# mynameisfiber/baton

Measured on NVIDIA H100. Metric: federated local samples/sec (whole box), ResNet-18 FedAvg, synthetic non-IID 32x32 shards, higher is better.
Workload: dtype bf16

## Files before the change

baton_b200/csrc/bindings.cpp:

```cpp
#include <ATen/cuda/CUDAContext.h>
#include <c10/cuda/CUDAGuard.h>
#include <torch/extension.h>

#include <optional>
#include <vector>

#include "launch.h"

namespace {

inline cudaStream_t cur_stream() { return at::cuda::getCurrentCUDAStream().stream(); }
inline void check(int rc, const char* what) {
  TORCH_CHECK(rc == 0, "baton_b200::", what, " failed with code ", rc,
              rc > 0 ? std::string(" (") + cudaGetErrorString(static_cast<cudaError_t>(rc)) + ")" : std::string());
}
inline const void* cptr(const at::Tensor& t) { return t.data_ptr(); }
inline void* ptr(at::Tensor& t) { return t.data_ptr(); }
template <class T>
inline T* opt_ptr(const std::optional<at::Tensor>& t) {
  return (t.has_value() && t->defined()) ? reinterpret_cast<T*>(t->data_ptr()) : nullptr;
}
#define CHECK_CUDA(x) TORCH_CHECK((x).is_cuda(), #x " must be a CUDA tensor")

inline const float* prox_anchor(const std::optional<at::Tensor>& anchor, int64_t numel, const at::Tensor& hyper) {
// ... 187 lines not shown
                    int64_t pad, int64_t ho, int64_t wo, int64_t cluster_k, int64_t force_bn,
                    const std::optional<at::Tensor>& col_stats, const std::optional<at::Tensor>& bn_scale,
                    const std::optional<at::Tensor>& bn_shift, const std::optional<at::Tensor>& residual, bool bn_relu) {
  CHECK_CUDA(x); CHECK_CUDA(w); CHECK_CUDA(y);
  TORCH_CHECK(x.scalar_type() == at::kBFloat16 && w.scalar_type() == at::kBFloat16 && y.scalar_type() == at::kBFloat16 &&
              x.dim() == 4 && x.is_contiguous() && w.is_contiguous() && y.is_contiguous());
  TORCH_CHECK(y.numel() == x.size(0) * ho * wo * w.size(0), "conv_igemm_fwd: y must hold [N*Ho*Wo, Cout] elements");
  const c10::cuda::CUDAGuard guard(x.device());
  const std::optional<B200AffineEpilogue> affine =
      affine_epilogue(bn_scale, bn_shift, residual, bn_relu, x.size(0) * ho * wo, w.size(0));
  const int rc = b200_conv_igemm_fwd(cptr(x), cptr(w), ptr(y), static_cast<int>(x.size(0)), static_cast<int>(x.size(1)),
                                     static_cast<int>(x.size(2)), static_cast<int>(x.size(3)), static_cast<int>(w.size(0)),
                                     static_cast<int>(kh), static_cast<int>(kw), static_cast<int>(stride),
                                     static_cast<int>(pad), static_cast<int>(ho), static_cast<int>(wo),
                                     static_cast<int>(cluster_k), static_cast<int>(force_bn), opt_ptr<float>(col_stats),
                                     affine ? &*affine : nullptr, cur_stream());
  if (rc == -2 || rc == B200_AFFINE_EPILOGUE_DECLINED) return false;
  check(rc, "conv_igemm_fwd");
  return true;
}
bool conv_igemm_dgrad(const at::Tensor& dy, const at::Tensor& w, at::Tensor dx, int64_t kh, int64_t kw, int64_t pad,
                      int64_t cluster_k, int64_t force_bn) {
  CHECK_CUDA(dy); CHECK_CUDA(w); CHECK_CUDA(dx);
  TORCH_CHECK(dy.scalar_type() == at::kBFloat16 && w.scalar_type() == at::kBFloat16 && dx.scalar_type() == at::kBFloat16 &&
              dy.dim() == 4 && dx.dim() == 4 && dy.is_contiguous() && w.is_contiguous() && dx.is_contiguous());
  const c10::cuda::CUDAGuard guard(dy.device());
  const int rc = b200_conv_igemm_dgrad(cptr(dy), cptr(w), ptr(dx), static_cast<int>(dx.size(0)), static_cast<int>(dx.size(1)),
                                       static_cast<int>(dx.size(2)), static_cast<int>(dx.size(3)), static_cast<int>(dy.size(3)),
                                       static_cast<int>(kh), static_cast<int>(kw), static_cast<int>(pad),
                                       static_cast<int>(dy.size(1)), static_cast<int>(dy.size(2)),
                                       static_cast<int>(cluster_k), static_cast<int>(force_bn), cur_stream());
  if (rc == -2) return false;
  check(rc, "conv_igemm_dgrad");
  return true;
}
bool conv_halo(const at::Tensor& src, const at::Tensor& w, at::Tensor out, bool dgrad, int64_t mc,
               const std::optional<at::Tensor>& col_stats) {
  CHECK_CUDA(src); CHECK_CUDA(w); CHECK_CUDA(out);
  TORCH_CHECK(src.scalar_type() == at::kBFloat16 && w.scalar_type() == at::kBFloat16 && out.scalar_type() == at::kBFloat16 &&
              src.dim() == 4 && src.size(3) == 64 && src.is_contiguous() && w.is_contiguous() && out.is_contiguous());
  const int64_t rows = src.size(0) * src.size(1) * src.size(2);
  TORCH_CHECK(rows > 0 && out.numel() % rows == 0, "conv_halo: out must hold [N*H*W, Nout] elements");
  const int64_t nout = out.numel() / rows;
  TORCH_CHECK(w.numel() == (dgrad ? 64 * 9 * nout : nout * 9 * 64), "conv_halo: w must be [Cout, 9*Cin]");
  TORCH_CHECK(dgrad ? !col_stats.has_value()
                    : (!col_stats.has_value() || (col_stats->scalar_type() == at::kFloat && col_stats->numel() >= 2 * nout)),
              "conv_halo: col_stats is a [2 Cout] fp32 buffer of the forward");
  const c10::cuda::CUDAGuard guard(src.device());
  const int rc = b200_conv_halo(cptr(src), cptr(w), ptr(out), static_cast<int>(src.size(0)), static_cast<int>(src.size(1)),
                                static_cast<int>(src.size(2)), static_cast<int>(nout), dgrad ? 1 : 0,
                                static_cast<int>(mc), opt_ptr<float>(col_stats), cur_stream());
  if (rc == -2) return false;
  check(rc, "conv_halo");
  return true;
}
bool conv_igemm_dgrad_s2(const at::Tensor& dy, const at::Tensor& w, at::Tensor dx, int64_t kh, int64_t kw,
                         const std::vector<int64_t>& ntaps, const std::vector<int64_t>& taps, int64_t force_bn) {
  CHECK_CUDA(dy); CHECK_CUDA(w); CHECK_CUDA(dx);
  TORCH_CHECK(dy.scalar_type() == at::kBFloat16 && w.scalar_type() == at::kBFloat16 && dx.scalar_type() == at::kBFloat16 &&
              dy.dim() == 4 && dx.dim() == 4 && dy.is_contiguous() && w.is_contiguous() && dx.is_contiguous());
  TORCH_CHECK(ntaps.size() == 4 && taps.size() == 16, "conv_igemm_dgrad_s2: 4 classes x 4 taps");
  int nt[4], tw[16];
  for (int i = 0; i < 4; ++i) nt[i] = static_cast<int>(ntaps[i]);
  for (int i = 0; i < 16; ++i) tw[i] = static_cast<int>(taps[i]);
  const c10::cuda::CUDAGuard guard(dy.device());
  const int rc = b200_conv_igemm_dgrad_s2(cptr(dy), cptr(w), ptr(dx), static_cast<int>(dx.size(0)),
                                          static_cast<int>(dx.size(1)), static_cast<int>(dx.size(2)),
                                          static_cast<int>(dx.size(3)), static_cast<int>(dy.size(3)), static_cast<int>(kh),
                                          static_cast<int>(kw), static_cast<int>(dy.size(1)), static_cast<int>(dy.size(2)),
                                          nt, tw, static_cast<int>(force_bn), cur_stream());
  if (rc == -2) return false;
  check(rc, "conv_igemm_dgrad_s2");
  return true;
}
bool conv_igemm_wgrad(const at::Tensor& dy, const at::Tensor& x, at::Tensor dw, int64_t cout, int64_t kh, int64_t kw,
                      int64_t stride, int64_t pad, int64_t ho, int64_t wo, int64_t split_k, int64_t force_bn,
                      const std::optional<at::Tensor>& sgd_theta, const std::optional<at::Tensor>& sgd_theta_bf16,
                      const std::optional<at::Tensor>& sgd_mom, const std::optional<at::Tensor>& sgd_hyper,
                      bool sgd_nesterov, const std::optional<at::Tensor>& sgd_anchor,
                      const std::optional<at::Tensor>& sgd_corr, const std::optional<at::Tensor>& sgd_v) {
  CHECK_CUDA(dy); CHECK_CUDA(x); CHECK_CUDA(dw);
  TORCH_CHECK(x.scalar_type() == at::kBFloat16 && dy.scalar_type() == at::kBFloat16 && dw.scalar_type() == at::kFloat &&
              x.dim() == 4 && x.is_contiguous() && dy.is_contiguous());
  const c10::cuda::CUDAGuard guard(x.device());
  const std::optional<B200SgdEpilogue> sgd =
      sgd_epilogue(sgd_theta, sgd_theta_bf16, sgd_mom, sgd_hyper, sgd_nesterov, sgd_anchor, sgd_corr, sgd_v);
  const int rc = b200_conv_igemm_wgrad(cptr(dy), cptr(x), dw.data_ptr<float>(), static_cast<int>(x.size(0)),
                                       static_cast<int>(x.size(1)), static_cast<int>(x.size(2)), static_cast<int>(x.size(3)),
                                       static_cast<int>(cout), static_cast<int>(kh), static_cast<int>(kw),
                                       static_cast<int>(stride), static_cast<int>(pad), static_cast<int>(ho),
                                       static_cast<int>(wo), static_cast<int>(split_k), static_cast<int>(force_bn),
                                       sgd ? &*sgd : nullptr, cur_stream());
  if (rc == -2 || rc == B200_SGD_EPILOGUE_DECLINED) return false;
  check(rc, "conv_igemm_wgrad");
  return true;
}

void gemm_fp8(const at::Tensor& a, const at::Tensor& b, at::Tensor d, const std::optional<at::Tensor>& bias,
              const std::optional<at::Tensor>& sfa, const std::optional<at::Tensor>& sfb, int64_t M, int64_t N, int64_t K,
              int64_t lda, int64_t ldb, int64_t ldd, int64_t act, int64_t split_k, bool accumulate, double alpha) {
  CHECK_CUDA(a); CHECK_CUDA(b); CHECK_CUDA(d);
  TORCH_CHECK(a.element_size() == 1 && b.element_size() == 1, "gemm_fp8 operands must be 1-byte (e4m3)");
  const c10::cuda::CUDAGuard guard(a.device());
  check(b200_gemm_fp8(cptr(a), cptr(b), ptr(d), opt_ptr<const float>(bias), opt_ptr<const void>(sfa),
                      opt_ptr<const void>(sfb), M, N, K, lda, ldb, ldd, d.scalar_type() == at::kFloat, act, split_k,
                      accumulate, static_cast<float>(alpha), cur_stream()),
// ... 758 lines not shown
                                       opt_ptr<float>(logits_out), static_cast<int>(x.size(0)), static_cast<int>(x.size(1)),
                                       static_cast<int>(w.size(0)), static_cast<float>(grad_scale), cur_stream());
  if (rc == -2) return false;
  check(rc, "linear_xent_head");
  return true;
}
bool linear_xent_eval(const at::Tensor& x, const at::Tensor& w, const std::optional<at::Tensor>& bias, const at::Tensor& target,
                      at::Tensor loss_acc, const std::optional<at::Tensor>& logits_out) {
  CHECK_CUDA(x);
  TORCH_CHECK(x.scalar_type() == at::kBFloat16 && w.scalar_type() == at::kBFloat16 && x.dim() == 2 && w.dim() == 2 &&
              x.is_contiguous() && w.is_contiguous() && x.size(1) == w.size(1));
  TORCH_CHECK(target.scalar_type() == at::kLong && target.numel() >= x.size(0) && loss_acc.scalar_type() == at::kFloat &&
              loss_acc.numel() >= 2);
  TORCH_CHECK(!bias.has_value() || (bias->scalar_type() == at::kFloat && bias->numel() == w.size(0)));
  TORCH_CHECK(!logits_out.has_value() || (logits_out->scalar_type() == at::kFloat && logits_out->is_contiguous() &&
                                          logits_out->numel() == x.size(0) * w.size(0)));
  const c10::cuda::CUDAGuard guard(x.device());
  const int rc = b200_linear_xent_eval(x.data_ptr(), w.data_ptr(), opt_ptr<const float>(bias),
                                       reinterpret_cast<const long long*>(target.data_ptr<int64_t>()),
                                       loss_acc.data_ptr<float>(), opt_ptr<float>(logits_out), static_cast<int>(x.size(0)),
                                       static_cast<int>(x.size(1)), static_cast<int>(w.size(0)), cur_stream());
  if (rc == -2) return false;
  check(rc, "linear_xent_eval");
  return true;
}
void mse(const at::Tensor& pred, const at::Tensor& target, const std::optional<at::Tensor>& dpred, at::Tensor loss_acc,
         double grad_scale) {
  CHECK_CUDA(pred);
  TORCH_CHECK(target.scalar_type() == at::kFloat && target.numel() == pred.numel());
  const c10::cuda::CUDAGuard guard(pred.device());
  const int in32 = pred.scalar_type() == at::kFloat;
  const int out32 = dpred.has_value() && dpred->defined() && dpred->scalar_type() == at::kFloat;
  check(b200_mse(pred.data_ptr(), in32, target.data_ptr<float>(), opt_ptr<void>(dpred), out32,
                 loss_acc.data_ptr<float>(), pred.numel(), static_cast<float>(grad_scale), cur_stream()),
        "mse");
}

}

PYBIND11_MODULE(TORCH_EXTENSION_NAME, m) {
  m.doc() = "baton_b200 sm_90a kernels";
  m.attr("MAX_RANKS") = B200_MAX_RANKS;
  m.def("gemm", &gemm);
  m.def("trace_set", &trace_set);
  m.def("attention_fwd", &attention_fwd);
  m.def("attention_bwd", &attention_bwd);
  m.def("bn_bwd_cluster", &bn_bwd_cluster);
  m.def("im2col_tma_probe", &im2col_tma_probe);
  m.def("conv_igemm_fwd", &conv_igemm_fwd);
  m.def("conv_igemm_wgrad", &conv_igemm_wgrad);
  m.def("conv_igemm_dgrad", &conv_igemm_dgrad);
  m.def("conv_igemm_dgrad_s2", &conv_igemm_dgrad_s2);
  m.def("conv_halo", &conv_halo);
  m.def("gemm_batched", &gemm_batched);
  m.def("gemm_fp8", &gemm_fp8);
  m.def("quant_mx_rows", &quant_mx_rows);
  m.def("quant_mx_cols", &quant_mx_cols);
  m.def("fused_sgd", &fused_sgd);
  m.def("fused_sgd_segments", &fused_sgd_segments);
  m.def("weighted_sum", &weighted_sum);
  m.def("fold_client", &fold_client);
  m.def("scaffold_corr", &scaffold_corr);
  m.def("scaffold_dc", &scaffold_dc);
  m.def("cast", &cast);
  m.def("gather_rows", &gather_rows);
  m.def("colsum", &colsum);
  m.def("add_bf16", &add_bf16);
  m.def("relu_bwd", &relu_bwd);
  m.def("gelu", &gelu);
  m.def("gelu_bwd", &gelu_bwd);
  m.def("pad_rows", &pad_rows);
  m.def("embedding_bwd", &embedding_bwd);
  m.def("fedavg_allreduce", &fedavg_allreduce);
  m.def("fedavg_allreduce_robust", &fedavg_allreduce_robust);
  m.def("fedavg_allreduce_krum", &fedavg_allreduce_krum);
  m.attr("KRUM_MAX_CTAS") = B200_KRUM_MAX_CTAS;
  m.attr("KRUM_PAIRS") = B200_KRUM_PAIRS;
  m.attr("KRUM_REPORT") = B200_KRUM_REPORT;
  m.def("fedavg_allreduce_topk", &fedavg_allreduce_topk);
  m.def("fedavg_allreduce_local", &fedavg_allreduce_local);
  m.def("topk_pack", &topk_pack);
  m.def("topk_fold", &topk_fold);
  m.def("nonzero_pack", &nonzero_pack);
  m.def("topk_work_words", [](int64_t n) { return static_cast<int64_t>(B200_TOPK_WORK_WORDS(n)); });
  m.def("pack_client", &pack_client);
  m.attr("MAX_ROBUST_CLIENTS") = B200_MAX_ROBUST_CLIENTS;
  m.attr("DP_WORK_WORDS") = B200_DP_WORK_WORDS;
  m.def("dp_clip_factor", &dp_clip_factor);
  m.def("fold_client_scaled", &fold_client_scaled);
  m.def("im2col", &im2col);
  m.def("col2im", &col2im);
  m.def("maxpool", &maxpool);
  m.def("maxpool_bwd", &maxpool_bwd);
  m.def("avgpool", &avgpool);
  m.def("avgpool_bwd", &avgpool_bwd);
  m.def("bn_stats", &bn_stats);
  m.def("bn_apply", &bn_apply);
  m.def("bn_bwd_reduce", &bn_bwd_reduce);
  m.def("bn_bwd_apply", &bn_bwd_apply);
  m.def("bn_relu_maxpool", &bn_relu_maxpool);
  m.def("bn_maxpool_bwd", &bn_maxpool_bwd);
  m.def("layernorm_fwd", &layernorm_fwd);
  m.def("layernorm_bwd", &layernorm_bwd);
  m.def("softmax_fwd", &softmax_fwd);
  m.def("softmax_bwd", &softmax_bwd);
  m.def("softmax_xent", &softmax_xent);
// ... 6 lines not shown
```

baton_b200/csrc/conv_halo.cu:

```cuda
#define B200_TU_TAG 12
#include "ptx.cuh"
#include "epilogue.cuh"
#include "launch.h"
#include "pdl.cuh"

namespace b200 {

constexpr int HALO_BM = 64;
constexpr int HALO_BN = 64;
constexpr int HALO_TAPS = 9;
constexpr int HALO_THREADS = 256;
constexpr int HALO_CONSUMERS = 128;
constexpr int HALO_SLOT_BYTES = 64 * 64 * 2;
constexpr int HALO_PART_PITCH = HALO_BN + 4;
constexpr int HALO_MAX_SMEM = 227 * 1024;

struct HaloParams {
  int M, N;
  int H, W;
  __nv_bfloat16* D;
  float* col_stats;
  int ncol;
  int mc;
  int halo_bytes;
// ... 92 lines not shown
    wgmma_wait<0>();
    wgmma_fence_operands(acc);
    if (threadIdx.x == 128) TRACE_POINT();

    named_bar_sync(1, HALO_CONSUMERS);
    float* part = reinterpret_cast<float*>(smem);
    wg_store_acc<HALO_BN>(acc, part, HALO_PART_PITCH, 0);
    named_bar_sync(1, HALO_CONSUMERS);
    const int q = ew & 1;
    const int c = (ew >> 1) * 32;
    const int lrow = q * 32 + lane;
    const int row = m0 + lrow;
    const int col0 = n0 + c;
    float* sstat = cstat + q * 2 * HALO_BN;
    const bool want_stats = p.col_stats != nullptr;
    if (col0 >= p.N) {
      if (want_stats) { sstat[c + lane] = 0.f; sstat[HALO_BN + c + lane] = 0.f; }
    } else {
      uint32_t r[32];
      acc_ld_row32(part + lrow * HALO_PART_PITCH + c, r);
      float v[32];
#pragma unroll
      for (int j = 0; j < 32; ++j) v[j] = __uint_as_float(r[j]);
      if (want_stats) stage_col_stats(sstat, HALO_BN, c, v);
      if (row < p.M) {
        __nv_bfloat16* d = p.D + static_cast<size_t>(row) * p.N + col0;
        if (col0 + 32 <= p.N && (p.N % 8) == 0) {
#pragma unroll
          for (int j = 0; j < 32; j += 8) {
            uint4 o;
            o.x = pack_bf16x2(v[j], v[j + 1]);
            o.y = pack_bf16x2(v[j + 2], v[j + 3]);
            o.z = pack_bf16x2(v[j + 4], v[j + 5]);
            o.w = pack_bf16x2(v[j + 6], v[j + 7]);
            *reinterpret_cast<uint4*>(d + j) = o;
          }
        } else {
          _Pragma("unroll") for (int j = 0; j < 32; ++j) if (col0 + j < p.N) d[j] = __float2bfloat16_rn(v[j]);
        }
      }
    }
    if (want_stats) {
      named_bar_sync(1, HALO_CONSUMERS);
      for (int i = threadIdx.x - 128; i < 2 * HALO_BN; i += HALO_CONSUMERS) {
        const int col = i < HALO_BN ? i : i - HALO_BN;
        if (n0 + col < p.N)
          atomicAdd(p.col_stats + (i < HALO_BN ? 0 : p.N) + n0 + col,
                    cstat[i] + cstat[2 * HALO_BN + i]);
      }
    }
  }
}

template <bool DGRAD>
static int launch_halo(const CUtensorMap& tx, const CUtensorMap& tw, const HaloParams& p, dim3 grid, int smem,
                cudaStream_t stream) {
  static bool configured = false;
  if (!configured) {
    cudaError_t e = cudaFuncSetAttribute(conv_halo_kernel<DGRAD>, cudaFuncAttributeMaxDynamicSharedMemorySize,
                                         HALO_MAX_SMEM);
    if (e != cudaSuccess) return static_cast<int>(e);
    configured = true;
  }
  cudaLaunchConfig_t cfg = {};
  cfg.gridDim = grid;
  cfg.blockDim = dim3(HALO_THREADS);
  cfg.dynamicSmemBytes = smem;
  cfg.stream = stream;
  cudaLaunchAttribute attr[2];
  int na = 0;
  if (pdl_enabled()) {
    attr[na].id = cudaLaunchAttributeProgrammaticStreamSerialization;
    attr[na].val.programmaticStreamSerializationAllowed = 1;
    ++na;
  }
  if (p.mc > 1) {
    attr[na].id = cudaLaunchAttributeClusterDimension;
    attr[na].val.clusterDim.x = 1;
    attr[na].val.clusterDim.y = p.mc;
    attr[na].val.clusterDim.z = 1;
    ++na;
  }
  cfg.attrs = attr;
  cfg.numAttrs = na;
  cudaError_t le = cudaLaunchKernelEx(&cfg, conv_halo_kernel<DGRAD>, tx, tw, p);
  if (le != cudaSuccess) return static_cast<int>(le);
  return static_cast<int>(cudaGetLastError());
}

}

extern "C" int b200_encode_map2_bf16(void* map, const void* base, long long rows, long long cols, long long ld,
                                     int box_cols, int box_rows);
extern "C" int b200_encode_map4_box_bf16(void* map, const void* base, const long long* dims,
                                         const long long* stride_bytes, const int* box);

extern "C" int b200_conv_halo(const void* src, const void* w, void* out, int N, int H, int W, int Nout, int dgrad, int mc,
                              float* col_stats, cudaStream_t stream) {
  using namespace b200;
  const long long M = static_cast<long long>(N) * H * W;
  if (M <= 0 || Nout <= 0) return 0;
  const int hw = H * W;
  const long long m_tiles = (M + HALO_BM - 1) / HALO_BM;
  if (hw <= 0 || HALO_BM % hw != 0 || H + 2 > 256 || W + 2 > 256 || M > (1ll << 30) || Nout % 8 != 0 ||
      (dgrad && Nout % 64 != 0) || (mc != 1 && mc != 2 && mc != 4) || m_tiles % mc != 0 ||
      (reinterpret_cast<uintptr_t>(src) & 15) || (reinterpret_cast<uintptr_t>(w) & 15) ||
      (reinterpret_cast<uintptr_t>(out) & 15))
    return -2;
  const int imgs = HALO_BM / hw;
  const int halo_bytes = (imgs * (H + 2) * (W + 2) * 128 + 1023) / 1024 * 1024;
  const int smem = halo_bytes + halo_fixed_bytes();
  if (smem > HALO_MAX_SMEM) return -2;
  CUtensorMap tx, tw;
  const long long dims[4] = {64, W, H, N};
  const long long strides[3] = {64 * 2, static_cast<long long>(W) * 64 * 2, static_cast<long long>(hw) * 64 * 2};
  const int box[4] = {64, W + 2, H + 2, imgs};
  int rc = b200_encode_map4_box_bf16(&tx, src, dims, strides, box);
  if (rc) return rc;
  const long long wrows = dgrad ? 64 : Nout, wcols = dgrad ? 9ll * Nout : 9ll * 64;
  rc = b200_encode_map2_bf16(&tw, w, wrows, wcols, wcols, 64, 64 / mc);
  if (rc) return rc;
  HaloParams p;
  p.M = static_cast<int>(M); p.N = Nout; p.H = H; p.W = W; p.D = reinterpret_cast<__nv_bfloat16*>(out);
  p.col_stats = col_stats; p.ncol = Nout; p.mc = mc; p.halo_bytes = halo_bytes;
  dim3 grid((Nout + HALO_BN - 1) / HALO_BN, static_cast<unsigned>(m_tiles), 1);
  return dgrad ? launch_halo<true>(tx, tw, p, grid, smem, stream) : launch_halo<false>(tx, tw, p, grid, smem, stream);
}

B200_TRACE_REGISTER(conv_halo)
```

baton_b200/csrc/launch.h:

```cpp
#pragma once
#include <cuda_runtime.h>
#include <stdint.h>

#define B200_MAX_RANKS 16

extern "C" {

struct B200SgdEpilogue {
  float* theta;
  void* theta_bf16;
  float* mom;
  const float* hyper;
  int nesterov;
  const float* anchor;
  const float* corr;
  float* v;
};
#define B200_SGD_EPILOGUE_DECLINED (-6)

struct B200AffineEpilogue {
  const float* scale;
  const float* shift;
  const void* residual;
  long long ldr;
  int relu;
};
#define B200_AFFINE_EPILOGUE_DECLINED (-7)

int b200_gemm_bf16(const void* a, const void* b, void* d, const float* bias, int M, int N, int K, long long lda,
                   long long ldb, long long ldd, int a_mn, int b_mn, int out_fp32, int act, int split_k, int accumulate,
                   float alpha, const uint32_t* tile_flags, uint32_t flag_epoch, long long flag_elem_off, int flag_tile_elems,
                   long long flag_bias_off, int force_bn, float* col_stats, const uint32_t* flag_epoch_ptr,
                   const B200SgdEpilogue* sgd, const B200AffineEpilogue* affine, cudaStream_t stream);
int b200_gemm_bf16_batched(const void* a, const void* b, void* d, int M, int N, int K, long long lda, long long ldb,
                           long long ldd, int a_mn, int b_mn, int out_fp32, int act, float alpha, int n_outer,
                           int n_inner, long long a_outer, long long a_inner, long long b_outer, long long b_inner,
                           long long d_outer, long long d_inner, int accumulate, cudaStream_t stream);
int b200_attention_fwd(const void* qkv, void* out, void* probs, int B, int S, int H, int dh, float scale,
                       cudaStream_t stream);
int b200_attention_bwd(const void* qkv, const void* dout, const void* probs, void* dqkv, int B, int S, int H, int dh,
                       float scale, cudaStream_t stream);
int b200_conv_igemm_fwd(const void* x, const void* w, void* y, int N, int H, int W, int Cin, int Cout, int KH, int KW,
                        int stride, int pad, int Ho, int Wo, int cluster_k, int force_bn, float* col_stats,
                        const B200AffineEpilogue* affine, cudaStream_t stream);
int b200_conv_igemm_dgrad(const void* dy, const void* w, void* dx, int N, int H, int W, int Cin, int Cout, int KH, int KW,
                          int pad, int Ho, int Wo, int cluster_k, int force_bn, cudaStream_t stream);
int b200_conv_igemm_dgrad_s2(const void* dy, const void* w, void* dx, int N, int H, int W, int Cin, int Cout, int KH,
                             int KW, int Ho, int Wo, const int* ntaps, const int* taps, int force_bn, cudaStream_t stream);
int b200_conv_igemm_wgrad(const void* dy, const void* x, float* dw, int N, int H, int W, int Cin, int Cout, int KH, int KW,
                          int stride, int pad, int Ho, int Wo, int split_k, int force_bn, const B200SgdEpilogue* sgd,
                          cudaStream_t stream);
int b200_conv_halo(const void* src, const void* w, void* out, int N, int H, int W, int Nout, int dgrad, int mc,
                   float* col_stats, cudaStream_t stream);
int b200_im2col_tma_probe(const void* x, void* col, int N, int H, int W, int C, int KH, int KW, int stride, int pad,
                          int Ho, int Wo, cudaStream_t stream);
int b200_gemm_fp8(const void* a, const void* b, void* d, const float* bias, const void* sfa, const void* sfb, int M, int N,
                  int K, long long lda, long long ldb, long long ldd, int out_fp32, int act, int split_k, int accumulate,
                  float alpha, cudaStream_t stream);
int b200_quant_mx_rows(const void* x, void* q, void* sf, long long R, int C, long long ld_in, int Cp, cudaStream_t stream);
int b200_quant_mx_cols(const void* x, void* q, void* sf, long long R, int C, long long ld_in, long long Rp,
                       cudaStream_t stream);
int b200_gemm_simt(const void* a, const void* b, void* d, const float* bias, int M, int N, int K, long long lda,
                   long long ldb, long long ldd, int a_mn, int b_mn, int out_fp32, int act, int accumulate,
                   float alpha, cudaStream_t stream);

int b200_fused_sgd(float* w, float* g, float* mom, void* w_bf16, long long n, const float* hyper, int zero_grad,
                   int nesterov, const unsigned long long* wire_slot, const float* pack_global,
                   const float* pack_scale, long long n_pack, int wire_fp32, const float* prox_anchor,
                   const float* corr, float* adam_v, cudaStream_t stream);
int b200_fused_sgd_segments(float* w, float* g, float* mom, void* w_bf16, const long long* segments, int n_seg,
                            const float* hyper, int nesterov, const float* prox_anchor, const float* corr,
                            float* adam_v, cudaStream_t stream);
int b200_scaffold_corr(float* corr, const float* c, const float* ci, long long n, cudaStream_t stream);
int b200_scaffold_dc(float* up, float* ci, const float* c, const float* global_w, const float* theta, long long n,
                     float inv_k_eta, int first, cudaStream_t stream);
int b200_fold_client(float* acc, float* theta, const float* global_w, void* w_bf16, float* mom, long long n_mom, long long n,
                     float nk, int mode, int reset, cudaStream_t stream);
int b200_weighted_sum(void* dst, const void* const* srcs, const float* weights, int n_src, long long n, int dtype,
                      cudaStream_t stream);
int b200_cast_f32_bf16(const float* src, void* dst, long long n, cudaStream_t stream);
int b200_cast_bf16_f32(const void* src, float* dst, long long n, cudaStream_t stream);
int b200_gather_rows(const void* src, const long long* idx, void* dst, long long n_rows, long long row_bytes,
                     cudaStream_t stream);
int b200_gather_rows_i64(const long long* src, const long long* idx, long long* dst, long long n,
                         cudaStream_t stream);
int b200_colsum(const void* x, float* out, long long rows, int cols, int accumulate, cudaStream_t stream);
int b200_add_bf16(const void* a, const void* b, void* out, long long n, int relu, cudaStream_t stream);
int b200_relu_bwd_bf16(const void* y, const void* dy, void* dx, long long n, cudaStream_t stream);
int b200_gelu_bf16(const void* x, void* y, long long n, cudaStream_t stream);
int b200_gelu_bwd_bf16(const void* x, const void* dy, void* dx, long long n, cudaStream_t stream);
int b200_embedding_bwd(const void* dy, const long long* idx, float* grad, long long n_rows, int width,
                       cudaStream_t stream);
int b200_pad_rows_bf16(const void* src, void* dst, long long rows, int k, int kp, const uint32_t* flags,
                       const uint32_t* epoch_word, long long elem_off, int granule, cudaStream_t stream);

struct FedAvgArgs {
  void* wire[B200_MAX_RANKS];
  unsigned long long* pads[B200_MAX_RANKS];
  void* wire_mc;
  float* theta;
  float* global_w;
  void* theta_bf16;
  float* momentum;
  long long n_momentum;
  long long* int_local;
  long long* int_wire[B200_MAX_RANKS];
// ... 145 lines not shown
```

baton_b200/ops/functional.py:

```python
from __future__ import annotations

import collections
import functools
from typing import List, Optional, Sequence, Tuple

import torch

from ._ext import load

BF16 = torch.bfloat16
NUM_SMS = 132


def _pitch(t: torch.Tensor) -> int:
    assert t.dim() == 2 and (t.stride(1) == 1 or t.shape[1] == 1), "GEMM operand must have unit inner stride"
    return t.stride(0) if t.shape[0] > 1 else max(t.stride(0), t.shape[1])


def _tma_ok(t: torch.Tensor) -> bool:
    return t.dtype == BF16 and _pitch(t) % 8 == 0 and t.data_ptr() % 16 == 0


def pick_bn(M: int, N: int) -> int:
    m_tiles = (M + 127) // 128
# ... 315 lines not shown


@functools.lru_cache(maxsize=None)
def conv_plan(n: int, h: int, w: int, c: int, cout: int, kh: int, kw: int, stride: int, pad: int) -> ConvPlan:
    ho, wo = conv_out_size(h, kh, stride, pad), conv_out_size(w, kw, stride, pad)
    tap = None
    if h == 1 and w == 1 and kh == kw and kh % 2 == 1 and kh > 1 and pad == kh // 2 and c % 8 == 0:
        form, K, tap = "centre", c, (kh // 2) * kw + kw // 2
    elif kh == 1 and kw == 1 and stride == 1 and pad == 0 and c % 8 == 0:
        form, K = "pointwise", c
    elif c % 64 == 0:
        form, K = "implicit", kh * kw * c
    else:
        form, K = "im2col", im2col_k(kh, kw, c)
    dgrad = "view" if form in ("centre", "pointwise") else "col2im"
    if form == "implicit" and (stride == 2 or (stride == 1 and kh == kw and kh > 1)):
        dgrad = "implicit"
    return ConvPlan(n, h, w, c, cout, kh, kw, stride, pad, form, ho, wo, n * ho * wo, K, tap, dgrad)


def conv_fwd(x: torch.Tensor, w2d: torch.Tensor, plan: ConvPlan, form: Optional[str] = None,
             col_stats: Optional[torch.Tensor] = None, gate: Optional[dict] = None,
             affine: Optional[dict] = None) -> Tuple[Optional[torch.Tensor], torch.Tensor]:
    form = form or plan.form
    if form == "implicit":
        return conv_igemm_fwd(x, w2d, plan.kh, plan.kw, plan.stride, plan.pad, col_stats=col_stats, affine=affine), x
    a = im2col(x, plan.kh, plan.kw, plan.stride, plan.pad)[0] if form == "im2col" else x.view(plan.M, plan.c)
    gk = {}
    if gate is not None and form != "centre":
        gk = dict(flags=gate["flags"], flag_epoch_word=gate["epoch_word"], flag_elem_off=gate["elem_off"],
                  flag_tile_elems=gate["tile_elems"], force_bn=pick_bn(a.shape[0], w2d.shape[0]))
    return gemm(a, plan.weight(w2d), col_stats=col_stats, affine=affine, **gk), a


HALO_BM = 64
_HALO_MAX_SMEM = 227 * 1024


def halo_smem_bytes(h: int, w: int) -> int:
    halo = round_up((HALO_BM // (h * w)) * (h + 2) * (w + 2) * 128, 1024)
    return halo + 9 * 8192 + 16 * 8 + 4 * 64 * 4 + 1024


def halo_eligible(kh: int, kw: int, stride: int, pad: int, c: int, h: int, w: int, affine: Optional[dict] = None) -> bool:
    return (kh == 3 and kw == 3 and stride == 1 and pad == 1 and c == 64 and h * w <= HALO_BM and
            HALO_BM % (h * w) == 0 and affine is None and halo_smem_bytes(h, w) <= _HALO_MAX_SMEM)


def halo_cluster(m_rows: int) -> int:
    tiles = (m_rows + HALO_BM - 1) // HALO_BM
    return 4 if tiles % 4 == 0 else 2 if tiles % 2 == 0 else 1


def _conv_path(path: Optional[str], eligible: bool) -> str:
    if path is None:
        return "halo" if eligible else "im2col"
    if path not in ("halo", "im2col"):
        raise ValueError("path must be None, 'halo' or 'im2col', not {!r}".format(path))
    if path == "halo" and not eligible:
        raise ValueError("the halo kernel does not take this convolution (see halo_eligible)")
    return path


def conv_igemm_fwd(x: torch.Tensor, w2d: torch.Tensor, kh: int, kw: int, stride: int, pad: int,
                   col_stats: Optional[torch.Tensor] = None, affine: Optional[dict] = None,
                   cluster_k: Optional[int] = None, force_bn: int = 0,
                   out: Optional[torch.Tensor] = None, path: Optional[str] = None,
                   mc: Optional[int] = None) -> Optional[torch.Tensor]:
    n, h, w, c = x.shape
    cout = w2d.shape[0]
    if c % 64 or w2d.shape[1] != kh * kw * c or not x.is_contiguous() or not w2d.is_contiguous():
        return None
    ho, wo = conv_out_size(h, kh, stride, pad), conv_out_size(w, kw, stride, pad)
    M, K = n * ho * wo, kh * kw * c
    if _conv_path(path, halo_eligible(kh, kw, stride, pad, c, h, w, affine) and cout % 8 == 0) == "halo":
        y = out if out is not None else torch.empty((M, cout), dtype=BF16, device=x.device)
        if not load().conv_halo(x, w2d, y, False, mc or halo_cluster(M), col_stats):
            raise RuntimeError("conv_halo declined a convolution halo_eligible admits")
        return y
    bn = force_bn or pick_bn(M, cout)
    if cluster_k is None:
        cluster_k = pick_cluster_k(M, cout, K, bn)
    y = out if out is not None else torch.empty((M, cout), dtype=BF16, device=x.device)
    af = affine or {}
    ok = load().conv_igemm_fwd(x, w2d, y, kh, kw, stride, pad, ho, wo, cluster_k, bn, col_stats, af.get("scale"),
                               af.get("shift"), af.get("residual"), bool(af.get("relu", False)))
    return y if ok else None


S2_MAX_TAPS = 4


def conv_s2_dgrad_taps(kh: int, kw: int, pad: int, ho: int, wo: int) -> Optional[List[List[Tuple[int, int, int]]]]:
    classes = []
    for a in (0, 1):
        for b in (0, 1):
            taps = []
            for r in range(kh):
                if (a + pad - r) % 2:
                    continue
                dp = (a + pad - r) // 2
                for s in range(kw):
                    if (b + pad - s) % 2:
                        continue
                    dq = (b + pad - s) // 2
                    if dp < 0 or dq < 0:
                        return None
                    if dp < ho and dq < wo:
                        taps.append((r * kw + s, dp, dq))
            if len(taps) > S2_MAX_TAPS:
                return None
            classes.append(taps)
    return classes


def conv_igemm_dgrad(dy: torch.Tensor, w2d: torch.Tensor, in_shape, kh: int, kw: int, pad: int, stride: int = 1,
                     out: Optional[torch.Tensor] = None, path: Optional[str] = None,
                     mc: Optional[int] = None) -> Optional[torch.Tensor]:
    n, h, w, c = in_shape
    cout = dy.shape[-1]
    if c % 64 or cout % 64 or w2d.shape[1] != kh * kw * c or not dy.is_contiguous() or not w2d.is_contiguous():
        return None
    if _conv_path(path, halo_eligible(kh, kw, stride, pad, cout, h, w)) == "halo":
        dx = out if out is not None else torch.empty((n, h, w, c), dtype=BF16, device=dy.device)
        if not load().conv_halo(dy, w2d, dx, True, mc or halo_cluster(n * h * w), None):
            raise RuntimeError("conv_halo declined a convolution halo_eligible admits")
        return dx
    if stride == 1:
        M, K = n * h * w, kh * kw * cout
        bn = pick_bn(M, c)
        dx = out if out is not None else torch.empty((n, h, w, c), dtype=BF16, device=dy.device)
        ok = load().conv_igemm_dgrad(dy, w2d, dx, kh, kw, pad, pick_cluster_k(M, c, K, bn), bn)
        return dx if ok else None
    if stride != 2:
        return None
    ho, wo = dy.shape[1], dy.shape[2]
    classes = conv_s2_dgrad_taps(kh, kw, pad, ho, wo)
    if classes is None:
        return None
    bn = pick_bn(4 * n * ho * wo, c)
    words = [[t | dp << 16 | dq << 24 for t, dp, dq in taps] + [0] * (S2_MAX_TAPS - len(taps)) for taps in classes]
    dx = out if out is not None else torch.empty((n, h, w, c), dtype=BF16, device=dy.device)
    ok = load().conv_igemm_dgrad_s2(dy, w2d, dx, kh, kw, [len(t) for t in classes], [x for ws in words for x in ws], bn)
    return dx if ok else None


def conv_igemm_wgrad_(dy2d: torch.Tensor, x: torch.Tensor, dw2d: torch.Tensor, kh: int, kw: int, stride: int,
                      pad: int, sgd: Optional[dict] = None) -> bool:
    n, h, w, c = x.shape
    cout = dy2d.shape[1]
    if c % 64 or not x.is_contiguous() or not dy2d.is_contiguous() or not dw2d.is_contiguous():
        return False
    ho, wo = conv_out_size(h, kh, stride, pad), conv_out_size(w, kw, stride, pad)
    M, K = n * ho * wo, kh * kw * c
    bn = pick_bn(cout, K)
    split_k = pick_split_k(cout, K, M, bn)
    if sgd is not None and split_k != 1:
        return False
    sg = sgd or {}
    return bool(load().conv_igemm_wgrad(dy2d, x, dw2d, cout, kh, kw, stride, pad, ho, wo, split_k, bn,
                                        sg.get("theta"), sg.get("theta_bf16"), sg.get("momentum"), sg.get("hyper"),
                                        bool(sg.get("nesterov", False)), sg.get("anchor"), sg.get("corr"),
                                        sg.get("adam_v")))


def col2im(col: torch.Tensor, shape: Tuple[int, int, int, int], kh: int, kw: int, stride: int, pad: int,
           ho: int, wo: int) -> torch.Tensor:
    n, h, w, c = shape
    dx = torch.empty(shape, dtype=BF16, device=col.device)
    load().col2im(col, dx, n, h, w, c, kh, kw, stride, pad, ho, wo, col.shape[1])
    return dx


def maxpool(x: torch.Tensor, k: int, stride: int, pad: int) -> Tuple[torch.Tensor, torch.Tensor]:
    n, h, w, c = x.shape
    ho, wo = conv_out_size(h, k, stride, pad), conv_out_size(w, k, stride, pad)
    y = torch.empty((n, ho, wo, c), dtype=BF16, device=x.device)
    arg = torch.empty((n, ho, wo, c), dtype=torch.uint8 if (c % 8 == 0 and k * k <= 255) else torch.int32, device=x.device)
    load().maxpool(x, y, arg, n, h, w, c, k, stride, pad, ho, wo)
    return y, arg


def maxpool_bwd(dy: torch.Tensor, arg: torch.Tensor, in_shape, k: int, stride: int, pad: int,
                dy_b: Optional[torch.Tensor] = None) -> torch.Tensor:
    n, h, w, c = in_shape
# ... 135 lines not shown
```

Baseline: 205,400.

## Add wide halo conv kernel for 128-channel stride-1 and 64-channel stride-2 3x3 convs

Adds a halo-based implicit-GEMM convolution kernel that also covers 128 input channels (two 64-channel halo blocks) and stride-2 forward with 64 channels. The whole input tile, padding included, is loaded into shared memory once by TMA, and all nine taps' weight tiles are loaded up front. The Python dispatcher sends these shapes to the new kernel by default, in place of the im2col igemm path. This is meant to remove im2col overhead and redundant input loads for later ResNet-18 layers with small spatial size. The cost is a large shared-memory footprint that allows one CTA per SM.

```diff
diff --git a/baton_b200/csrc/bindings.cpp b/baton_b200/csrc/bindings.cpp
--- a/baton_b200/csrc/bindings.cpp
+++ b/baton_b200/csrc/bindings.cpp
@@ -263,6 +263,29 @@
                                 static_cast<int>(mc), opt_ptr<float>(col_stats), cur_stream());
   if (rc == -2) return false;
   check(rc, "conv_halo");
+  return true;
+}
+bool conv_halo_wide(const at::Tensor& src, const at::Tensor& w, at::Tensor out, int64_t stride, bool dgrad, int64_t mc,
+                    const std::optional<at::Tensor>& col_stats) {
+  CHECK_CUDA(src); CHECK_CUDA(w); CHECK_CUDA(out);
+  TORCH_CHECK(src.scalar_type() == at::kBFloat16 && w.scalar_type() == at::kBFloat16 && out.scalar_type() == at::kBFloat16 &&
+              src.dim() == 4 && src.is_contiguous() && w.is_contiguous() && out.is_contiguous());
+  TORCH_CHECK(stride == 1 || stride == 2, "conv_halo_wide: stride 1 or 2");
+  const int64_t c = src.size(3);
+  const int64_t rows = src.size(0) * ((src.size(1) - 1) / stride + 1) * ((src.size(2) - 1) / stride + 1);
+  TORCH_CHECK(rows > 0 && out.numel() % rows == 0, "conv_halo_wide: out must hold [N*Ho*Wo, Nout] elements");
+  const int64_t nout = out.numel() / rows;
+  TORCH_CHECK(w.numel() == (dgrad ? c * 9 * nout : nout * 9 * c), "conv_halo_wide: w must be [Cout, 9*Cin]");
+  TORCH_CHECK(dgrad ? !col_stats.has_value()
+                    : (!col_stats.has_value() || (col_stats->scalar_type() == at::kFloat && col_stats->numel() >= 2 * nout)),
+              "conv_halo_wide: col_stats is a [2 Cout] fp32 buffer of the forward");
+  const c10::cuda::CUDAGuard guard(src.device());
+  const int rc = b200_conv_halo_wide(cptr(src), cptr(w), ptr(out), static_cast<int>(src.size(0)),
+                                     static_cast<int>(src.size(1)), static_cast<int>(src.size(2)), static_cast<int>(c),
+                                     static_cast<int>(nout), static_cast<int>(stride), dgrad ? 1 : 0,
+                                     static_cast<int>(mc), opt_ptr<float>(col_stats), cur_stream());
+  if (rc == -2) return false;
+  check(rc, "conv_halo_wide");
   return true;
 }
 bool conv_igemm_dgrad_s2(const at::Tensor& dy, const at::Tensor& w, at::Tensor dx, int64_t kh, int64_t kw,
@@ -1127,6 +1150,7 @@
   m.def("conv_igemm_dgrad", &conv_igemm_dgrad);
   m.def("conv_igemm_dgrad_s2", &conv_igemm_dgrad_s2);
   m.def("conv_halo", &conv_halo);
+  m.def("conv_halo_wide", &conv_halo_wide);
   m.def("gemm_batched", &gemm_batched);
   m.def("gemm_fp8", &gemm_fp8);
   m.def("quant_mx_rows", &quant_mx_rows);
diff --git a/baton_b200/csrc/conv_halo.cu b/baton_b200/csrc/conv_halo.cu
--- a/baton_b200/csrc/conv_halo.cu
+++ b/baton_b200/csrc/conv_halo.cu
@@ -168,12 +168,12 @@
   }
 }
 
-template <bool DGRAD>
-static int launch_halo(const CUtensorMap& tx, const CUtensorMap& tw, const HaloParams& p, dim3 grid, int smem,
+template <auto KERNEL, typename Params>
+static int launch_halo(const CUtensorMap& tx, const CUtensorMap& tw, const Params& p, dim3 grid, int smem,
                 cudaStream_t stream) {
   static bool configured = false;
   if (!configured) {
-    cudaError_t e = cudaFuncSetAttribute(conv_halo_kernel<DGRAD>, cudaFuncAttributeMaxDynamicSharedMemorySize,
+    cudaError_t e = cudaFuncSetAttribute(KERNEL, cudaFuncAttributeMaxDynamicSharedMemorySize,
                                          HALO_MAX_SMEM);
     if (e != cudaSuccess) return static_cast<int>(e);
     configured = true;
@@ -199,7 +199,7 @@
   }
   cfg.attrs = attr;
   cfg.numAttrs = na;
-  cudaError_t le = cudaLaunchKernelEx(&cfg, conv_halo_kernel<DGRAD>, tx, tw, p);
+  cudaError_t le = cudaLaunchKernelEx(&cfg, KERNEL, tx, tw, p);
   if (le != cudaSuccess) return static_cast<int>(le);
   return static_cast<int>(cudaGetLastError());
 }
@@ -240,7 +240,211 @@
   p.M = static_cast<int>(M); p.N = Nout; p.H = H; p.W = W; p.D = reinterpret_cast<__nv_bfloat16*>(out);
   p.col_stats = col_stats; p.ncol = Nout; p.mc = mc; p.halo_bytes = halo_bytes;
   dim3 grid((Nout + HALO_BN - 1) / HALO_BN, static_cast<unsigned>(m_tiles), 1);
-  return dgrad ? launch_halo<true>(tx, tw, p, grid, smem, stream) : launch_halo<false>(tx, tw, p, grid, smem, stream);
+  return dgrad ? launch_halo<conv_halo_kernel<true>>(tx, tw, p, grid, smem, stream)
+               : launch_halo<conv_halo_kernel<false>>(tx, tw, p, grid, smem, stream);
+}
+
+namespace b200 {
+
+struct HaloWideParams {
+  int M, N;
+  int Ho, Wo;
+  __nv_bfloat16* D;
+  float* col_stats;
+  int ncol;
+  int mc;
+  int halo_bytes;
+};
+
+__host__ __device__ constexpr int halo_wide_fixed_bytes(int k_tiles) {
+  return k_tiles * HALO_SLOT_BYTES + 32 * 8 + 4 * HALO_BN * 4 + 1024;
+}
+
+template <bool DGRAD, int CB, int STRIDE>
+__global__ void __launch_bounds__(HALO_THREADS, 1)
+conv_halo_wide_kernel(const __grid_constant__ CUtensorMap tmX, const __grid_constant__ CUtensorMap tmW,
+                      const HaloWideParams p) {
+  constexpr int KT = HALO_TAPS * CB;
+  static_assert(1 + KT <= 32, "one mbarrier per k-tile");
+  extern __shared__ __align__(1024) uint8_t smem_raw[];
+  uint8_t* smem = reinterpret_cast<uint8_t*>((reinterpret_cast<uintptr_t>(smem_raw) + 1023) & ~uintptr_t(1023));
+  uint8_t* halo = smem;
+  uint8_t* bslot = smem + CB * p.halo_bytes;
+  uint64_t* bar = reinterpret_cast<uint64_t*>(bslot + KT * HALO_SLOT_BYTES);
+  float* cstat = reinterpret_cast<float*>(bar + 32);
+
+  griddep_launch_dependents();
+  const int warp = threadIdx.x >> 5;
+  const int m0 = blockIdx.y * HALO_BM;
+  const int n0 = blockIdx.x * HALO_BN;
+  const int hw = p.Ho * p.Wo;
+  const int hp = STRIDE * (p.Ho - 1) + 3, wp = STRIDE * (p.Wo - 1) + 3;
+
+  if (warp == 0 && elect_one()) {
+    tma_prefetch_desc(&tmX);
+    tma_prefetch_desc(&tmW);
+    for (int i = 0; i < 1 + KT; ++i) mbar_init(&bar[i], 1);
+    fence_barrier_init();
+  }
+  __syncthreads();
+  if (p.mc > 1) cluster_sync_all();
+  griddep_wait();
+
+  if (warp == 0) {
+    if (elect_one()) {
+      const int imgs = HALO_BM / hw;
+      mbar_expect_tx(&bar[0], CB * imgs * hp * wp * 128);
+#pragma unroll
+      for (int cb = 0; cb < CB; ++cb) tma_load_4d(halo + cb * p.halo_bytes, &tmX, &bar[0], 64 * cb, -1, -1, m0 / hw);
+      const int rows = 64 / p.mc;
+      const int rank = p.mc > 1 ? static_cast<int>(cluster_ctarank()) : 0;
+      const uint16_t mask = static_cast<uint16_t>((1u << p.mc) - 1);
+#pragma unroll 1
+      for (int kt = 0; kt < KT; ++kt) {
+        const int tap = kt / CB, cb = kt - tap * CB;
+        mbar_expect_tx(&bar[1 + kt], HALO_SLOT_BYTES);
+        uint8_t* dst = bslot + kt * HALO_SLOT_BYTES + rank * rows * 128;
+        const int c0 = DGRAD ? (HALO_TAPS - 1 - tap) * p.ncol + n0 : kt * 64;
+        const int c1 = DGRAD ? cb * 64 + rank * rows : n0 + rank * rows;
+        if (p.mc > 1)
+          tma_load_2d_mc(dst, &tmW, &bar[1 + kt], c0, c1, mask);
+        else
+          tma_load_2d(dst, &tmW, &bar[1 + kt], c0, c1);
+      }
+    }
+  } else if (warp >= 4) {
+    const int ew = warp - 4;
+    const int lane = static_cast<int>(lane_id());
+    const int m = 16 * ew + (lane & 15);
+    const int img = m / hw, rem = m - img * hw;
+    const int oi = rem / p.Wo, oj = rem - oi * p.Wo;
+    const int hrow0 = (img * hp + STRIDE * oi) * wp + STRIDE * oj;
+    const uint32_t halo_a = smem_u32(halo);
+    const int half = lane >> 4;
+    auto load_a = [&](uint32_t (&a)[4][4], int kt) {
+      const int tap = kt / CB, cb = kt - tap * CB;
+      const int r = tap / 3, s = tap - 3 * r;
+      const int hrow = hrow0 + r * wp + s;
+      const uint32_t row_addr = halo_a + static_cast<uint32_t>(cb * p.halo_bytes + hrow * 128);
+#pragma unroll
+      for (int kk = 0; kk < 4; ++kk) ldmatrix_x4(a[kk], row_addr + ((((2 * kk + half) ^ hrow) & 7) << 4));
+    };
+
+    float acc[32];
+#pragma unroll
+    for (int j = 0; j < 32; ++j) acc[j] = 0.f;
+    uint32_t a[2][4][4];
+    mbar_wait(&bar[0], 0);
+    load_a(a[0], 0);
+#pragma unroll
+    for (int kt = 0; kt < KT; ++kt) {
+      mbar_wait(&bar[1 + kt], 0);
+      const uint32_t sb = smem_u32(bslot + kt * HALO_SLOT_BYTES);
+      wgmma_fence();
+#pragma unroll
+      for (int kk = 0; kk < 4; ++kk) {
+        const uint64_t bd = DGRAD ? gmma_desc_sw128(sb + kk * 2048, 8192, 1024) : gmma_desc_sw128(sb + kk * 32, 16, 1024);
+        wgmma_bf16_n64_rs<DGRAD ? 1 : 0>(acc, a[kt & 1][kk], bd, 1u);
+      }
+      wgmma_commit();
+      if (kt + 1 < KT) {
+        wgmma_wait<1>();
+        load_a(a[(kt + 1) & 1], kt + 1);
+      }
+    }
+    wgmma_wait<0>();
+    wgmma_fence_operands(acc);
+    if (threadIdx.x == 128) TRACE_POINT();
+
+    named_bar_sync(1, HALO_CONSUMERS);
+    float* part = reinterpret_cast<float*>(smem);
+    wg_store_acc<HALO_BN>(acc, part, HALO_PART_PITCH, 0);
+    named_bar_sync(1, HALO_CONSUMERS);
+    const int q = ew & 1;
+    const int c = (ew >> 1) * 32;
+    const int lrow = q * 32 + lane;
+    const int row = m0 + lrow;
+    const int col0 = n0 + c;
+    float* sstat = cstat + q * 2 * HALO_BN;
+    const bool want_stats = p.col_stats != nullptr;
+    if (col0 >= p.N) {
+      if (want_stats) { sstat[c + lane] = 0.f; sstat[HALO_BN + c + lane] = 0.f; }
+    } else {
+      uint32_t r[32];
+      acc_ld_row32(part + lrow * HALO_PART_PITCH + c, r);
+      float v[32];
+#pragma unroll
+      for (int j = 0; j < 32; ++j) v[j] = __uint_as_float(r[j]);
+      if (want_stats) stage_col_stats(sstat, HALO_BN, c, v);
+      if (row < p.M) {
+        __nv_bfloat16* d = p.D + static_cast<size_t>(row) * p.N + col0;
+        if (col0 + 32 <= p.N && (p.N % 8) == 0) {
+#pragma unroll
+          for (int j = 0; j < 32; j += 8) {
+            uint4 o;
+            o.x = pack_bf16x2(v[j], v[j + 1]);
+            o.y = pack_bf16x2(v[j + 2], v[j + 3]);
+            o.z = pack_bf16x2(v[j + 4], v[j + 5]);
+            o.w = pack_bf16x2(v[j + 6], v[j + 7]);
+            *reinterpret_cast<uint4*>(d + j) = o;
+          }
+        } else {
+          _Pragma("unroll") for (int j = 0; j < 32; ++j) if (col0 + j < p.N) d[j] = __float2bfloat16_rn(v[j]);
+        }
+      }
+    }
+    if (want_stats) {
+      named_bar_sync(1, HALO_CONSUMERS);
+      for (int i = threadIdx.x - 128; i < 2 * HALO_BN; i += HALO_CONSUMERS) {
+        const int col = i < HALO_BN ? i : i - HALO_BN;
+        if (n0 + col < p.N)
+          atomicAdd(p.col_stats + (i < HALO_BN ? 0 : p.N) + n0 + col,
+                    cstat[i] + cstat[2 * HALO_BN + i]);
+      }
+    }
+  }
+}
+
+}
+
+extern "C" int b200_conv_halo_wide(const void* src, const void* w, void* out, int N, int H, int W, int C, int Nout,
+                                   int stride, int dgrad, int mc, float* col_stats, cudaStream_t stream) {
+  using namespace b200;
+  const bool s2 = stride == 2 && C == 64 && !dgrad, s1 = stride == 1 && C == 128;
+  if (!s2 && !s1) return -2;
+  const int Ho = (H - 1) / stride + 1, Wo = (W - 1) / stride + 1;
+  const long long M = static_cast<long long>(N) * Ho * Wo;
+  if (M <= 0 || Nout <= 0) return 0;
+  const int hw = Ho * Wo;
+  const long long m_tiles = (M + HALO_BM - 1) / HALO_BM;
+  const int hp = stride * (Ho - 1) + 3, wp = stride * (Wo - 1) + 3;
+  if (H <= 0 || W <= 0 || HALO_BM % hw != 0 || hp > 256 || wp > 256 || M > (1ll << 30) || Nout % 8 != 0 ||
+      (dgrad && Nout % 64 != 0) || (mc != 1 && mc != 2 && mc != 4 && mc != 8) || m_tiles % mc != 0 ||
+      (reinterpret_cast<uintptr_t>(src) & 15) || (reinterpret_cast<uintptr_t>(w) & 15) ||
+      (reinterpret_cast<uintptr_t>(out) & 15))
+    return -2;
+  const int imgs = HALO_BM / hw;
+  const int cb = C / 64;
+  const int halo_bytes = (imgs * hp * wp * 128 + 1023) / 1024 * 1024;
+  const int smem = cb * halo_bytes + halo_wide_fixed_bytes(HALO_TAPS * cb);
+  if (smem > HALO_MAX_SMEM) return -2;
+  CUtensorMap tx, tw;
+  const long long dims[4] = {C, W, H, N};
+  const long long strides[3] = {static_cast<long long>(C) * 2, static_cast<long long>(W) * C * 2,
+                                static_cast<long long>(H) * W * C * 2};
+  const int box[4] = {64, wp, hp, imgs};
+  int rc = b200_encode_map4_box_bf16(&tx, src, dims, strides, box);
+  if (rc) return rc;
+  const long long wrows = dgrad ? C : Nout, wcols = dgrad ? 9ll * Nout : 9ll * C;
+  rc = b200_encode_map2_bf16(&tw, w, wrows, wcols, wcols, 64, 64 / mc);
+  if (rc) return rc;
+  HaloWideParams p;
+  p.M = static_cast<int>(M); p.N = Nout; p.Ho = Ho; p.Wo = Wo; p.D = reinterpret_cast<__nv_bfloat16*>(out);
+  p.col_stats = col_stats; p.ncol = Nout; p.mc = mc; p.halo_bytes = halo_bytes;
+  dim3 grid((Nout + HALO_BN - 1) / HALO_BN, static_cast<unsigned>(m_tiles), 1);
+  if (s2) return launch_halo<conv_halo_wide_kernel<false, 1, 2>>(tx, tw, p, grid, smem, stream);
+  return dgrad ? launch_halo<conv_halo_wide_kernel<true, 2, 1>>(tx, tw, p, grid, smem, stream)
+               : launch_halo<conv_halo_wide_kernel<false, 2, 1>>(tx, tw, p, grid, smem, stream);
 }
 
 B200_TRACE_REGISTER(conv_halo)
diff --git a/baton_b200/csrc/launch.h b/baton_b200/csrc/launch.h
--- a/baton_b200/csrc/launch.h
+++ b/baton_b200/csrc/launch.h
@@ -52,6 +52,8 @@
                           cudaStream_t stream);
 int b200_conv_halo(const void* src, const void* w, void* out, int N, int H, int W, int Nout, int dgrad, int mc,
                    float* col_stats, cudaStream_t stream);
+int b200_conv_halo_wide(const void* src, const void* w, void* out, int N, int H, int W, int C, int Nout, int stride,
+                        int dgrad, int mc, float* col_stats, cudaStream_t stream);
 int b200_im2col_tma_probe(const void* x, void* col, int N, int H, int W, int C, int KH, int KW, int stride, int pad,
                           int Ho, int Wo, cudaStream_t stream);
 int b200_gemm_fp8(const void* a, const void* b, void* d, const float* bias, const void* sfa, const void* sfb, int M, int N,
diff --git a/baton_b200/ops/functional.py b/baton_b200/ops/functional.py
--- a/baton_b200/ops/functional.py
+++ b/baton_b200/ops/functional.py
@@ -391,13 +391,31 @@
     return 4 if tiles % 4 == 0 else 2 if tiles % 2 == 0 else 1
 
 
+_HALO_WIDE_FORMS = ((1, 128), (2, 64))
+
+
+def halo_wide_smem_bytes(c: int, h: int, w: int, stride: int) -> int:
+    ho, wo = conv_out_size(h, 3, stride, 1), conv_out_size(w, 3, stride, 1)
+    box = (HALO_BM // (ho * wo)) * (stride * (ho - 1) + 3) * (stride * (wo - 1) + 3) * 128
+    return c // 64 * (round_up(box, 1024) + 9 * 8192) + 32 * 8 + 4 * 64 * 4 + 1024
+
+
+def halo_wide_eligible(kh: int, kw: int, stride: int, pad: int, c: int, h: int, w: int,
+                       affine: Optional[dict] = None, dgrad: bool = False) -> bool:
+    if kh != 3 or kw != 3 or pad != 1 or (stride, c) not in _HALO_WIDE_FORMS or (dgrad and stride != 1):
+        return False
+    hw = conv_out_size(h, 3, stride, 1) * conv_out_size(w, 3, stride, 1)
+    return (hw <= HALO_BM and HALO_BM % hw == 0 and affine is None and
+            halo_wide_smem_bytes(c, h, w, stride) <= _HALO_MAX_SMEM)
+
+
 def _conv_path(path: Optional[str], eligible: bool) -> str:
     if path is None:
         return "halo" if eligible else "im2col"
     if path not in ("halo", "im2col"):
         raise ValueError("path must be None, 'halo' or 'im2col', not {!r}".format(path))
     if path == "halo" and not eligible:
-        raise ValueError("the halo kernel does not take this convolution (see halo_eligible)")
+        raise ValueError("no halo kernel takes this convolution (see halo_eligible, halo_wide_eligible)")
     return path
 
 
@@ -412,10 +430,14 @@
         return None
     ho, wo = conv_out_size(h, kh, stride, pad), conv_out_size(w, kw, stride, pad)
     M, K = n * ho * wo, kh * kw * c
-    if _conv_path(path, halo_eligible(kh, kw, stride, pad, c, h, w, affine) and cout % 8 == 0) == "halo":
+    halo = halo_eligible(kh, kw, stride, pad, c, h, w, affine) and cout % 8 == 0
+    wide = halo_wide_eligible(kh, kw, stride, pad, c, h, w, affine) and cout % 8 == 0
+    if _conv_path(path, halo or wide) == "halo":
         y = out if out is not None else torch.empty((M, cout), dtype=BF16, device=x.device)
-        if not load().conv_halo(x, w2d, y, False, mc or halo_cluster(M), col_stats):
+        if halo and not load().conv_halo(x, w2d, y, False, mc or halo_cluster(M), col_stats):
             raise RuntimeError("conv_halo declined a convolution halo_eligible admits")
+        if wide and not load().conv_halo_wide(x, w2d, y, stride, False, mc or halo_cluster(M), col_stats):
+            raise RuntimeError("conv_halo_wide declined a convolution halo_wide_eligible admits")
         return y
     bn = force_bn or pick_bn(M, cout)
     if cluster_k is None:
@@ -455,21 +477,27 @@
 
 def conv_igemm_dgrad(dy: torch.Tensor, w2d: torch.Tensor, in_shape, kh: int, kw: int, pad: int, stride: int = 1,
                      out: Optional[torch.Tensor] = None, path: Optional[str] = None,
-                     mc: Optional[int] = None) -> Optional[torch.Tensor]:
+                     mc: Optional[int] = None, cluster_k: Optional[int] = None) -> Optional[torch.Tensor]:
     n, h, w, c = in_shape
     cout = dy.shape[-1]
     if c % 64 or cout % 64 or w2d.shape[1] != kh * kw * c or not dy.is_contiguous() or not w2d.is_contiguous():
         return None
-    if _conv_path(path, halo_eligible(kh, kw, stride, pad, cout, h, w)) == "halo":
+    halo = halo_eligible(kh, kw, stride, pad, cout, h, w)
+    wide = halo_wide_eligible(kh, kw, stride, pad, cout, h, w, dgrad=True)
+    if _conv_path(path, halo or wide) == "halo":
         dx = out if out is not None else torch.empty((n, h, w, c), dtype=BF16, device=dy.device)
-        if not load().conv_halo(dy, w2d, dx, True, mc or halo_cluster(n * h * w), None):
+        if halo and not load().conv_halo(dy, w2d, dx, True, mc or halo_cluster(n * h * w), None):
             raise RuntimeError("conv_halo declined a convolution halo_eligible admits")
+        if wide and not load().conv_halo_wide(dy, w2d, dx, 1, True, mc or halo_cluster(n * h * w), None):
+            raise RuntimeError("conv_halo_wide declined a convolution halo_wide_eligible admits")
         return dx
     if stride == 1:
         M, K = n * h * w, kh * kw * cout
         bn = pick_bn(M, c)
         dx = out if out is not None else torch.empty((n, h, w, c), dtype=BF16, device=dy.device)
-        ok = load().conv_igemm_dgrad(dy, w2d, dx, kh, kw, pad, pick_cluster_k(M, c, K, bn), bn)
+        if cluster_k is None:
+            cluster_k = pick_cluster_k(M, c, K, bn)
+        ok = load().conv_igemm_dgrad(dy, w2d, dx, kh, kw, pad, cluster_k, bn)
         return dx if ok else None
     if stride != 2:
         return None
```

New measurement: 225,600, median of 6. +9.8%, better.
